# Plachtaa/FAcodec

Measured on NVIDIA H100. Metric: audio_seconds_per_second, higher is better.
Workload: dtype f32 I/O and accumulation; every product is a 3-MMA split of fp32 operands: fp16 hi + 2^11-scaled fp16 lo (22 mantissa bits, register-promoted accumulation) upstream of the VQ, bf16 hi + bf16 lo (16 bits) downstream

## Files before the change

### facodec_b200/_lib.py

```python
import ctypes
import os

from . import build as _build

_c = ctypes
_LIB = None


class FacError(RuntimeError):
    pass


def lib_path():
    return _build.LIB


def load():
    global _LIB
    if _LIB is not None:
        return _LIB
    path = lib_path()
    if not os.path.exists(path):
        raise FacError(f"{path} not found: build it with `python -m facodec_b200.build` "
                       "(needs nvcc; there is no CPU fallback)")
    L = ctypes.CDLL(path)
    vp, i32, i64p, fp = _c.c_void_p, _c.c_int, _c.c_void_p, _c.c_void_p
    sigs = {
        "fac_abi_version": ([], i32),
        "fac_create": ([_c.POINTER(vp), i32], i32),
        "fac_destroy": ([vp], i32),
        "fac_last_error": ([vp], _c.c_char_p),
        "fac_load_tensor": ([vp, i32, _c.c_char_p, fp, _c.POINTER(_c.c_int64), i32], i32),
        "fac_finalize": ([vp], i32),
        "fac_encode": ([vp, fp, i32, i32, fp, vp], i32),
        "fac_encode_frames": ([i32], i32),
        "fac_quantize": ([vp, fp, fp, i32, i32, i32, i32, fp, i32, i64p, fp, fp, fp, fp, fp, fp, i64p, i64p, i64p, vp], i32),
        "fac_decode": ([vp, fp, i32, i32, fp, vp], i32),
        "fac_codec_forward": ([vp, fp, i32, i32, i32, fp, i64p, i64p, i64p, fp, vp], i32),
        "fac_codec_forward_host": ([vp, fp, i32, i32, i32, fp, i64p, i64p, i64p, vp], i32),
        "fac_codec_encode": ([vp, fp, i32, i32, i32, i64p, i64p, i64p, fp, vp], i32),
        "fac_codec_encode_lens": ([vp, fp, i32, i32, vp, i32, i64p, i64p, i64p, fp, vp], i32),
        "fac_codec_forward_lens": ([vp, fp, i32, i32, vp, i32, fp, i64p, i64p, i64p, fp, vp], i32),
        "fac_codec_timbre_lens": ([vp, fp, i32, i32, vp, fp, vp], i32),
        "fac_dequantize": ([vp, i64p, i64p, i32, i64p, i32, fp, i32, i32, fp, fp, fp, fp, vp], i32),
        "fac_codes_decode": ([vp, i64p, i64p, i32, i64p, i32, fp, i32, i32, fp, vp], i32),
        "fac_codes_decode_lens": ([vp, i64p, i64p, i32, i64p, i32, fp, i32, i32, vp, fp, vp], i32),
        "fac_redecode": ([vp, i64p, i64p, i32, fp, i32, i32, i32, i32, i32, fp, vp], i32),
        "fac_redecoder_decode": ([vp, fp, i32, i32, fp, vp], i32),
        "fac_voice_convert": ([vp, i64p, i64p, i32, fp, i32, i32, i32, i32, i32, fp, vp], i32),
        "fac_voice_convert_lens": ([vp, i64p, i64p, i32, fp, i32, i32, i32, i32, i32, vp, fp, vp], i32),
        "fac_dataset_mel": ([vp, fp, i32, i32, fp, vp], i32),
        "fac_head_begin": ([vp], i32),
        "fac_head_tensor": ([vp, i32, _c.c_char_p, fp, _c.POINTER(_c.c_int64), i32], i32),
        "fac_head_finalize": ([vp, i32, i32, i32, i32, i32], i32),
        "fac_head_forward": ([vp, i32, fp, i32, i32, _c.POINTER(vp), vp], i32),
        "fac_rvq_create": ([vp, i32] + [_c.POINTER(vp)] * 5, i32),
        "fac_rvq_destroy": ([vp, i32], i32),
        "fac_stream_begin": ([vp, i32], i32),
        "fac_stream_encode": ([vp, i32, fp, i32, fp, vp], i32),
        "fac_stream_decode": ([vp, i32, fp, i32, fp, vp], i32),
        "fac_stream_decode_codes": ([vp, i32, i64p, i64p, i32, i64p, i32, fp, i32, fp, vp], i32),
        "fac_stream_encode_codes": ([vp, i32, fp, i32, i32, i64p, i64p, i64p, vp], i32),
        "fac_stream_finish_codes": ([vp, i32, i64p, i64p, i64p, fp, vp], i32),
        "fac_stream_timbre": ([vp, i32, fp, vp], i32),
        "fac_stream_end": ([vp, i32], i32),
        "fac_vc_stream_lookahead": ([], i32),
        "fac_vc_stream_begin": ([vp, i32, fp, i32, i32, i32, vp], i32),
        "fac_vc_stream_convert": ([vp, i32, i64p, i64p, i32, i32, fp, vp], i32),
        "fac_vc_stream_finish": ([vp, i32, fp, vp], i32),
        "fac_vc_stream_set_timbre": ([vp, i32, fp, vp], i32),
        "fac_vc_stream_end": ([vp, i32], i32),
        "fac_codes_pool_create": ([vp, i32, i32], i32),
        "fac_codes_pool_open": ([vp, i32, vp], i32),
        "fac_codes_pool_encode_codes": ([vp, i32, i32, vp, vp, vp, vp, vp, vp, vp, vp], i32),
        "fac_codes_pool_finish_codes": ([vp, i32, i32, vp, vp, vp, vp, vp, vp], i32),
        "fac_codes_pool_timbre": ([vp, i32, i32, vp, vp, vp], i32),
        "fac_codes_pool_close": ([vp, i32, i32], i32),
        "fac_codes_pool_destroy": ([vp, i32], i32),
        "fac_vc_pool_create": ([vp, i32, i32, i32, i32], i32),
        "fac_vc_pool_open": ([vp, i32, fp, vp], i32),
        "fac_vc_pool_open_mode": ([vp, i32, fp, i32, i32, i32, vp], i32),
        "fac_vc_pool_set_timbre": ([vp, i32, i32, fp, vp], i32),
        "fac_vc_pool_convert": ([vp, i32, i32, vp, vp, vp, vp, vp, vp, vp, vp], i32),
        "fac_vc_pool_finish": ([vp, i32, i32, vp, vp, vp, vp], i32),
        "fac_vc_pool_close": ([vp, i32, i32], i32),
        "fac_vc_pool_destroy": ([vp, i32], i32),
        "fac_dec_pool_create": ([vp, i32], i32),
        "fac_dec_pool_open": ([vp, i32, fp, vp], i32),
        "fac_dec_pool_decode_codes": ([vp, i32, i32, vp, vp, vp, vp, vp, vp, vp, vp, vp], i32),
        "fac_dec_pool_set_timbre": ([vp, i32, i32, fp, vp], i32),
        "fac_dec_pool_close": ([vp, i32, i32], i32),
        "fac_dec_pool_destroy": ([vp, i32], i32),
        "fac_resample_geometry": ([i32, i32, _c.POINTER(_c.c_int)], i32),
        "fac_resample_out_len": ([i32, i32, _c.c_longlong], _c.c_longlong),
        "fac_resample_ready": ([i32, i32, i32, _c.c_longlong, _c.c_longlong], _c.c_longlong),
        "fac_resample_table": ([vp, i32, i32, fp], i32),
        "fac_resample": ([vp, fp, i32, i32, vp, i32, i32, fp, vp], i32),
        "fac_rs_pool_create": ([vp, i32, i32], i32),
        "fac_rs_pool_open": ([vp, i32, i32, i32], i32),
        "fac_rs_pool_push": ([vp, i32, i32, vp, vp, vp, vp, vp, vp], i32),
        "fac_rs_pool_finish": ([vp, i32, i32, vp, vp, vp, vp, vp, vp], i32),
        "fac_rs_pool_undo": ([vp, i32, i32, vp], i32),
        "fac_rs_pool_close": ([vp, i32, i32], i32),
        "fac_rs_pool_destroy": ([vp, i32], i32),
# ... 68 lines not shown
```

### facodec_b200/build.py

```python
import os
import subprocess
import sys

HERE = os.path.dirname(os.path.abspath(__file__))
CSRC = os.path.join(HERE, "csrc")
OUT_DIR = os.path.join(HERE, "_C")
LIB = os.path.join(OUT_DIR, "libfacodec_b200.so")
SOURCES = ["engine.cu", "conv_simt.cu", "conv_tc.cu", "lstm.cu", "lstm2.cu", "frontend.cu", "quant.cu", "altfree.cu", "pool.cu", "resample.cu"]
HEADERS = ["common.cuh", "kernels.h", "conv_tc_common.cuh", "resample.h", os.path.join("..", "..", "include", "facodec_b200.h"),
           os.path.join("..", "..", "include", "facodec_b200_debug.h")]
NVCC_FLAGS = ["-O3", "-std=c++17", "-lineinfo", "-gencode", "arch=compute_90a,code=sm_90a",
              "-Xcompiler", "-fPIC", "-Xcompiler", "-O3", "--expt-relaxed-constexpr"]


def _nvcc():
    for c in (os.environ.get("NVCC"), "/usr/local/cuda/bin/nvcc", "nvcc"):
        if c and (os.path.isabs(c) and os.path.exists(c) or not os.path.isabs(c)):
            return c
    return "nvcc"


def is_stale():
    if not os.path.exists(LIB):
        return True
    t = os.path.getmtime(LIB)
    deps = [os.path.join(CSRC, s) for s in SOURCES + HEADERS] + [os.path.abspath(__file__)]
    return any(os.path.getmtime(d) > t for d in deps if os.path.exists(d))


def build(force=False, verbose=False):
    if not force and not is_stale():
        return LIB
    os.makedirs(OUT_DIR, exist_ok=True)
    objs = []
    procs = []
    for s in SOURCES:
        obj = os.path.join(OUT_DIR, s.replace(".cu", ".o"))
        cmd = [_nvcc()] + NVCC_FLAGS + (["-Xptxas", "-v"] if verbose else []) + ["-c", os.path.join(CSRC, s), "-o", obj]
        procs.append((s, subprocess.Popen(cmd, stdout=subprocess.PIPE, stderr=subprocess.STDOUT, text=True)))
        objs.append(obj)
    fail = False
    for s, p in procs:
        out, _ = p.communicate()
        if p.returncode != 0 or verbose:
            sys.stderr.write(f"--- {s} ---\n{out}\n")
        fail |= p.returncode != 0
    if fail:
        raise RuntimeError("nvcc failed")
    cmd = [_nvcc(), "-shared", "-o", LIB] + objs + ["-gencode", "arch=compute_90a,code=sm_90a", "-lcudart"]
    subprocess.check_call(cmd)
    return LIB


if __name__ == "__main__":
    print(build(force="--force" in sys.argv, verbose="-v" in sys.argv))
```

### facodec_b200/csrc/conv_tc.cu

```cuda
#include <cuda_bf16.h>
#include <cuda_fp16.h>

#include <cstring>
#include <mutex>
#include <type_traits>

#include "common.cuh"
#include "conv_tc_common.cuh"
#include "kernels.h"

namespace fac {

namespace {

using namespace tc;

enum Prec { P_TF32 = 0, P_BF16 = 1, P_F16S = 2, P_F16X2 = 3, P_NONE = -1 };

template <int P> struct PrecT {
    static constexpr int KG = P == P_TF32 ? 4 : 2;
    static constexpr int planes = P == P_F16S ? 1 : 2;
    static constexpr int ksteps = P == P_TF32 ? 2 : 1;
    static constexpr int kind = P == P_TF32 ? WG_TF32 : (P == P_BF16 ? WG_BF16 : WG_F16);
};

__host__ __device__ constexpr int prec_kg(int P) { return P == P_TF32 ? 4 : 2; }
__host__ __device__ constexpr int prec_planes(int P) { return P == P_F16S ? 1 : 2; }
__host__ __device__ constexpr uint32_t master_bytes(bool promoted, int nchunk, int promote_every, int ni) {
    return promoted && nchunk > promote_every ? (uint32_t)ni / 2 * 4 * kThreads : 0u;
}

template <int NI>
__device__ __forceinline__ void zero_acc(float (&a)[NI / 2]) {
#pragma unroll
    for (int i = 0; i < NI / 2; ++i) a[i] = 0.f;
}

template <int P, int NI>
__device__ __forceinline__ void mma_pass(float (&acc)[NI / 2], uint32_t a_addr, uint32_t a_lbo, uint32_t b_addr,
                                         uint32_t b_lbo) {
#pragma unroll
    for (int ks = 0; ks < PrecT<P>::ksteps; ++ks)
        wgmma_ss<NI, PrecT<P>::kind>(acc, gdesc(a_addr + ks * 2 * a_lbo, a_lbo, 128), gdesc(b_addr + ks * 2 * b_lbo, b_lbo, 128));
}

struct Tile {
    int row0, col0, nw;
    int warp, lane;
};

template <int NI, int GROUP = NI, typename F>
__device__ __forceinline__ void for_each_pair(const Tile& tl, const float (&acc)[NI / 2], F&& f) {
#pragma unroll
    for (int j = 0; j < NI / 8; ++j) {
        if (j > 0 && (8 * j) % GROUP == 0 && 8 * j >= tl.nw) break;
#pragma unroll
        for (int h = 0; h < 2; ++h) {
            const int row = tl.row0 + 16 * tl.warp + (tl.lane >> 2) + 8 * h;
            const int col = tl.col0 + 8 * j + 2 * (tl.lane & 3);
            f(row, col, acc[4 * j + 2 * h], acc[4 * j + 2 * h + 1]);
        }
    }
}

template <bool FAST>
__device__ __forceinline__ float act_out(int act, float v, float al, float ia) {
    if (act == ACT_SNAKE) return FAST ? fmaf(ia, sin2_mufu(al * v), v) : snake_fast(v, al, ia);
    if (act == ACT_TANH) return tanhf(v);
    if (act == ACT_MISH) return mish_f(v);
    return v;
}

template <int P1, int P2, bool TT>
constexpr bool groupable() { return P1 != P_F16S && P2 == P_NONE && !TT; }

template <int P1, int P2, bool PROMO, int NI, int MINB = 1, bool TT = false>
__global__ void __launch_bounds__(kThreads, groupable<P1, P2, TT>() && NI <= 128 ? 2 : MINB) conv_tc_kernel(TcConvParams p) {
    constexpr bool FUSED = P2 != P_NONE;
    constexpr bool GROUPABLE = groupable<P1, P2, TT>();
    static_assert(!TT || (NI == 64 && !FUSED), "transposed tiles: <= 64 channels x 64 time steps per warpgroup");
    static_assert(NI % 16 == 0 && NI <= (PROMO || MINB == 2 ? 64 : (P1 == P_F16S ? 256 : 128)),
                  "accumulator registers: <= 64 / 128 columns (256 in the one-pass fp16 class at one CTA per SM)");
    constexpr bool F16X2 = P1 == P_F16X2;
    constexpr bool DEC = P1 == P_BF16 || P1 == P_F16S;
    using T1 = PrecT<P1>;
    extern __shared__ __align__(1024) uint8_t smem[];
    uint64_t* full = reinterpret_cast<uint64_t*>(smem);

    const int tid = threadIdx.x, wg = tid >> 7;
    const int BM = 64 * p.MT;
    const int N = p.N, NW = p.MT == 2 ? N : N / 2;
    Tile tl;
    tl.row0 = p.MT == 2 ? 64 * wg : 0;
    tl.col0 = p.MT == 2 ? 0 : wg * NW;
    tl.nw = NW;
    tl.warp = (tid >> 5) & 3;
    tl.lane = tid & 31;
    const int t0 = blockIdx.x * BM, ntile = blockIdx.y, b = blockIdx.z;
    const int Kr = p.Kr, dil = p.dil, Rpad = p.Rpad, nchunk = p.nchunk, S = p.stagesB;
    const int G = GROUPABLE ? p.group : 1;
    const int R = BM + (Kr - 1) * dil;
    const int nstep1 = G == 4 ? nchunk >> 2 : (G == 2 ? nchunk >> 1 : nchunk);
    const uint32_t a_plane = (uint32_t)G * T1::KG * Rpad * 16, a_bytes = a_plane * T1::planes;
    uint8_t* abuf = smem + kSmemHdr;
    float4* master = reinterpret_cast<float4*>(abuf + 2 * (size_t)a_bytes);
    const uint32_t m_bytes = master_bytes(PROMO, nchunk, p.promote_every, NI);
    uint8_t* wbuf = abuf + 2 * (size_t)a_bytes + m_bytes;
    uint8_t* a2buf = m_bytes ? reinterpret_cast<uint8_t*>(master) : wbuf + (size_t)S * p.b_slot;
    const uint32_t w_unit1 = (uint32_t)Kr * T1::planes * T1::KG * N * 16;
    const uint32_t w_unit2 = FUSED ? (uint32_t)prec_planes(P2) * prec_kg(P2) * N * 16 : 0;
    const int units = nstep1 + (FUSED ? p.nchunk2 : 0);

    if (tid == 0) {
        for (int i = 0; i < S; ++i) mbar_init(&full[i], 1);
        fence_mbar_init();
    }
    __syncthreads();
    auto issue_w = [&](int u) {
        uint64_t* bar = &full[u % S];
        uint8_t* dst = wbuf + (size_t)(u % S) * p.b_slot;
        const uint8_t* src;
        uint32_t bytes;
        if (u < nstep1) {
            src = reinterpret_cast<const uint8_t*>(p.wblob) + ((size_t)ntile * nchunk + (size_t)u * G) * w_unit1;
            bytes = G * w_unit1;
        } else { src = reinterpret_cast<const uint8_t*>(p.wblob2) + (size_t)(u - nstep1) * w_unit2; bytes = w_unit2; }
        mbar_arrive_expect_tx(bar, bytes);
        bulk_g2s(dst, src, bytes, bar);
    };
    if (tid == 0)
        for (int u = 0; u < S - 1 && u < units; ++u) issue_w(u);

    const PadMap pm = PadMap::lane(p.lane_len, b, p.Tin, p.pad_left_s, p.pad_right_s, p.reflect);
    const float* __restrict__ xb = p.x + (size_t)b * p.x_bstride;
    auto produce = [&](int s) {
        uint8_t* ahi = abuf + (size_t)(s & 1) * a_bytes;
        auto run = [&](auto grouped) {
            constexpr bool GR = decltype(grouped)::value;
            const int c = GR ? s * G : s;
            if constexpr (P1 == P_TF32) produce_chunk<kThreads, GR, false>(p, pm, xb, c, G, t0, R, Rpad, ahi, ahi + a_plane, tid);
            else if constexpr (P1 == P_BF16) produce_chunk<kThreads, GR, true>(p, pm, xb, c, G, t0, R, Rpad, ahi, ahi + a_plane, tid);
            else if constexpr (P1 == P_F16S) produce_chunk<kThreads, GR, true, 4, false, false, true>(p, pm, xb, c, G, t0, R, Rpad, ahi, ahi, tid);
            else produce_chunk<kThreads, GR, false, 4, false, true>(p, pm, xb, c, G, t0, R, Rpad, ahi, ahi + a_plane, tid);
        };
        if constexpr (GROUPABLE) {
            if (G > 1) run(std::true_type());
            else run(std::false_type());
        } else {
            run(std::false_type());
        }
        fence_proxy_async();
    };
    produce(0);

    float acc[NI / 2];
    float crs[F16X2 ? NI / 2 : 1];
    zero_acc<NI>(acc);
    if constexpr (F16X2) zero_acc<NI>(crs);
    const uint32_t a_lbo = (uint32_t)Rpad * 16, b_lbo = (uint32_t)N * 16;
    const uint32_t abase = smem_u32(abuf), wbase = smem_u32(wbuf), a2base = smem_u32(a2buf);
    const int BM2 = BM;

    auto promote = [&](bool first, bool last) {
        if constexpr (PROMO) {
#pragma unroll
            for (int q = 0; q < NI / 8; ++q) {
                float w[4];
#pragma unroll
                for (int e = 0; e < 4; ++e) {
                    const int i = 4 * q + e;
                    if constexpr (F16X2) { w[e] = acc[i] + crs[i] * kLoUnscale; crs[i] = 0.f; }
                    else w[e] = acc[i];
                }
                float4 m = first ? make_float4(0.f, 0.f, 0.f, 0.f) : master[q * kThreads + tid];
                m.x += w[0]; m.y += w[1]; m.z += w[2]; m.w += w[3];
                if (!last) master[q * kThreads + tid] = m;
                acc[4 * q + 0] = last ? m.x : 0.f;
                acc[4 * q + 1] = last ? m.y : 0.f;
                acc[4 * q + 2] = last ? m.z : 0.f;
                acc[4 * q + 3] = last ? m.w : 0.f;
            }
        }
    };

#pragma unroll 1
    for (int u = 0; u < units; ++u) {
        __syncthreads();
        if (tid == 0 && u + S - 1 < units) issue_w(u + S - 1);
        mbar_wait(&full[u % S], (uint32_t)(u / S) & 1u);
        const uint32_t wslot = wbase + (uint32_t)(u % S) * p.b_slot;
        wg_fence();
        if (u < nstep1) {
            const uint32_t a0 = abase + (uint32_t)(u & 1) * a_bytes + (uint32_t)tl.row0 * 16;
            const uint32_t b0 = wslot + (uint32_t)tl.col0 * 16;
            auto mma_tap = [&](uint32_t ahi, uint32_t bhi) {
                const uint32_t alo = ahi + a_plane, blo = bhi + T1::KG * b_lbo;
                if constexpr (TT) {
                    mma_pass<P1, NI>(acc, bhi, b_lbo, ahi, a_lbo);
                    mma_pass<P1, NI>(crs, bhi, b_lbo, alo, a_lbo);
                    mma_pass<P1, NI>(crs, blo, b_lbo, ahi, a_lbo);
                } else if constexpr (P1 == P_F16S) {
                    mma_pass<P1, NI>(acc, ahi, a_lbo, bhi, b_lbo);
                } else if constexpr (F16X2) {
                    mma_pass<P1, NI>(acc, ahi, a_lbo, bhi, b_lbo);
                    mma_pass<P1, NI>(crs, ahi, a_lbo, blo, b_lbo);
                    mma_pass<P1, NI>(crs, alo, a_lbo, bhi, b_lbo);
                } else {
                    mma_pass<P1, NI>(acc, ahi, a_lbo, bhi, b_lbo);
                    mma_pass<P1, NI>(acc, ahi, a_lbo, blo, b_lbo);
                    mma_pass<P1, NI>(acc, alo, a_lbo, bhi, b_lbo);
                }
            };
            if constexpr (GROUPABLE) {
                uint32_t ac = a0, bc = b0, ahi = a0, bhi = b0;
#pragma unroll 1
                for (int i = 0, tap = 0; i < G * Kr; ++i) {
                    mma_tap(ahi, bhi);
                    if (++tap < Kr) { ahi += (uint32_t)dil * 16; bhi += T1::planes * T1::KG * b_lbo; }
                    else { tap = 0; ac += T1::KG * a_lbo; bc += w_unit1; ahi = ac; bhi = bc; }
                }
            } else {
#pragma unroll 1
                for (int tap = 0; tap < Kr; ++tap)
                    mma_tap(a0 + (uint32_t)(tap * dil) * 16, b0 + (uint32_t)tap * T1::planes * T1::KG * b_lbo);
            }
            wg_commit();
            if (u + 1 < nstep1) produce(u + 1);
            wg_wait_all();
            const int done = (u + 1) * G;
            if (PROMO && (done % p.promote_every == 0 || done == nchunk)) promote(done <= p.promote_every, done == nchunk);
            if constexpr (FUSED) {
                if (u + 1 == nstep1) {
                    constexpr int KG2 = prec_kg(P2 < 0 ? 0 : P2);
                    const uint32_t a2_plane = (uint32_t)(p.nchunk2 * KG2) * BM2 * 16;
                    if (m_bytes) __syncthreads();
                    for_each_pair<NI, 32>(tl, acc, [&](int row, int col, float v0, float v1) {
                        const float2 bi = __ldg(reinterpret_cast<const float2*>(p.bias + col));
                        const float2 al = __ldg(reinterpret_cast<const float2*>(p.out_alpha + col));
                        const float2 ia = __ldg(reinterpret_cast<const float2*>(p.out_inv_alpha + col));
                        v0 = act_out<DEC>(ACT_SNAKE, v0 + bi.x, al.x, ia.x);
                        v1 = act_out<DEC>(ACT_SNAKE, v1 + bi.y, al.y, ia.y);
                        if constexpr (P2 == P_BF16) {
                            __nv_bfloat162 h = __floats2bfloat162_rn(v0, v1);
                            float2 hf = __bfloat1622float2(h);
                            __nv_bfloat162 l = __floats2bfloat162_rn(v0 - hf.x, v1 - hf.y);
                            const uint32_t off = ((uint32_t)(col >> 3) * BM2 + row) * 16 + (col & 7) * 2;
                            *reinterpret_cast<__nv_bfloat162*>(a2buf + off) = h;
                            *reinterpret_cast<__nv_bfloat162*>(a2buf + a2_plane + off) = l;
                        } else if constexpr (P2 == P_F16X2) {
                            const __half2 h = __floats2half2_rn(v0, v1);
                            const float2 hf = __half22float2(h);
                            const __half2 l = __floats2half2_rn((v0 - hf.x) * kLoScale, (v1 - hf.y) * kLoScale);
                            const uint32_t off = ((uint32_t)(col >> 3) * BM2 + row) * 16 + (col & 7) * 2;
                            *reinterpret_cast<__half2*>(a2buf + off) = h;
                            *reinterpret_cast<__half2*>(a2buf + a2_plane + off) = l;
                        } else {
                            const float h0 = to_tf32(v0), h1 = to_tf32(v1);
                            const uint32_t off = ((uint32_t)(col >> 2) * BM2 + row) * 16 + (col & 3) * 4;
                            *reinterpret_cast<float2*>(a2buf + off) = make_float2(h0, h1);
                            *reinterpret_cast<float2*>(a2buf + a2_plane + off) = make_float2(to_tf32(v0 - h0), to_tf32(v1 - h1));
                        }
                    });
                    fence_proxy_async();
                    zero_acc<NI>(acc);
                }
            }
        } else if constexpr (FUSED) {
            constexpr int P2x = P2 < 0 ? 0 : P2;
            constexpr int KG2 = prec_kg(P2x);
            const int c2 = u - nstep1;
            const uint32_t a2_plane = (uint32_t)(p.nchunk2 * KG2) * BM2 * 16, a2_lbo = (uint32_t)BM2 * 16;
            const uint32_t ahi = a2base + ((uint32_t)(c2 * KG2) * BM2 + tl.row0) * 16, alo = ahi + a2_plane;
            const uint32_t bhi = wslot + (uint32_t)tl.col0 * 16, blo = bhi + KG2 * b_lbo;
            if constexpr (P2x == P_F16X2) {
                mma_pass<P2x, NI>(acc, ahi, a2_lbo, bhi, b_lbo);
                mma_pass<P2x, NI>(crs, ahi, a2_lbo, blo, b_lbo);
                mma_pass<P2x, NI>(crs, alo, a2_lbo, bhi, b_lbo);
            } else {
                mma_pass<P2x, NI>(acc, ahi, a2_lbo, bhi, b_lbo);
                mma_pass<P2x, NI>(acc, ahi, a2_lbo, blo, b_lbo);
                mma_pass<P2x, NI>(acc, alo, a2_lbo, bhi, b_lbo);
            }
            wg_commit();
            wg_wait_all();
            if (PROMO && c2 + 1 == p.nchunk2) promote(true, true);
        }
    }

    const float* __restrict__ bias = FUSED ? p.bias2 : p.bias;
    const int act = FUSED ? ACT_NONE : p.out_act;
    float* __restrict__ yb = p.y + (size_t)b * p.y_bstride + (size_t)ntile * N;
    const float* __restrict__ rb = p.res ? p.res + (size_t)b * p.y_bstride + (size_t)ntile * N : nullptr;
    const float* al_p = act == ACT_SNAKE ? p.out_alpha + (size_t)ntile * N : nullptr;
    const float* ia_p = act == ACT_SNAKE ? p.out_inv_alpha + (size_t)ntile * N : nullptr;
    const float* bi_p = bias ? bias + (size_t)ntile * N : nullptr;
    if constexpr (TT) {
        for_each_pair<NI>(tl, acc, [&](int r, int c, float v0, float v1) {
            if (r - tl.row0 >= NW) return;
            const int co = tl.col0 + (r - tl.row0), tf = tl.row0 + (c - tl.col0);
            const float bi = bi_p ? __ldg(bi_p + co) : 0.f;
            const float al = act == ACT_SNAKE ? __ldg(al_p + co) : 0.f, ia = act == ACT_SNAKE ? __ldg(ia_p + co) : 0.f;
            const float v[2] = {v0, v1};
#pragma unroll
            for (int e = 0; e < 2; ++e) {
                const int t = t0 + tf + e;
                if (t >= p.Tout) continue;
                float o = act_out<DEC>(act, v[e] + bi, al, ia);
                if (rb) o += rb[(size_t)t * p.ldy + co];
                yb[(size_t)t * p.ldy + co] = o;
            }
        });
        return;
    }
    for_each_pair<NI>(tl, acc, [&](int row, int col, float v0, float v1) {
        const int t = t0 + row;
        if (t >= p.Tout) return;
        if (bi_p) { const float2 bi = __ldg(reinterpret_cast<const float2*>(bi_p + col)); v0 += bi.x; v1 += bi.y; }
        if (act == ACT_SNAKE) {
            const float2 al = __ldg(reinterpret_cast<const float2*>(al_p + col));
            const float2 ia = __ldg(reinterpret_cast<const float2*>(ia_p + col));
            v0 = act_out<DEC>(ACT_SNAKE, v0, al.x, ia.x);
            v1 = act_out<DEC>(ACT_SNAKE, v1, al.y, ia.y);
        } else if (act != ACT_NONE) {
            v0 = act_out<DEC>(act, v0, 0.f, 0.f);
            v1 = act_out<DEC>(act, v1, 0.f, 0.f);
        }
        if (rb) { const float2 r = *reinterpret_cast<const float2*>(rb + (size_t)t * p.ldy + col); v0 += r.x; v1 += r.y; }
        *reinterpret_cast<float2*>(yb + (size_t)t * p.ldy + col) = make_float2(v0, v1);
    });
}

}

namespace {
constexpr size_t kSmemCap = 227 * 1024;
constexpr size_t kSmemCap2 = 113 * 1024;
int plan_prec(const TcConvParams& p) {
    return p.g1f16 ? P_F16S : (p.f16x2 ? P_F16X2 : (p.bf16 ? P_BF16 : P_TF32));
}
constexpr int f16s_wide_nw(bool fused) { return fused ? 192 : 256; }
}

bool tc_conv_plan(TcConvParams& p) {
    if ((p.Cin % 4) != 0 || ((p.Cin * p.vf) % kChunk) != 0 || (p.Cout % 16) != 0) return false;
    if (p.bf16 && p.promoted) return false;
    if (p.f16x2 && !p.promoted) return false;
    if (p.g1f16 && !p.bf16) return false;
    if (p.tt && !p.f16x2) return false;
    if (p.fused && ((p.promoted && (!p.f16x2 || p.tt)) || p.Cin != p.Cout || p.vf != 1 || p.Cout > 256)) return false;
    const int P1 = plan_prec(p), P2 = p.fused ? (p.f16x2 ? P_F16X2 : (p.bf16 ? P_BF16 : P_TF32)) : P_NONE;
    p.nchunk = p.Cin * p.vf / kChunk;
    p.nchunk2 = p.fused ? p.Cout / kChunk : 0;
    p.promote_every = p.promoted ? (p.f16x2 ? (48 / p.Kr < 1 ? 1 : 48 / p.Kr) : (8 / p.Kr < 1 ? 1 : 8 / p.Kr)) : 1;
    if (p.fused && p.promoted && p.nchunk2 > 48) return false;
    const int nw_max = p.promoted ? 64 : 128;
    constexpr size_t kAReserve = 40 * 1024;
    int N = 0;
    for (int cand = p.fused ? p.Cout : 256; cand >= 16 && N == 0; cand -= 16) {
        const bool rows_split = cand <= nw_max, cols_split = (cand / 2) % 16 == 0 && cand / 2 <= nw_max;
        if (p.Cout % cand || !(rows_split || cols_split)) continue;
        size_t slot = (size_t)p.Kr * prec_planes(P1) * prec_kg(P1) * cand * 16, a2 = 0;
        if (P2 != P_NONE) a2 = (size_t)prec_planes(P2) * p.nchunk2 * prec_kg(P2) * 64 * 16;
        if (kSmemHdr + kAReserve + slot + a2 <= kSmemCap) N = cand;
        else if (p.fused) return false;
    }
    if (N == 0 || (p.fused && p.promoted && N != p.Cout)) return false;
    struct Layout { int Rpad; size_t slot, total; };
    auto layout = [&](int S, int MT, int G) {
        const int NW = MT == 2 ? N : N / 2, BM = 64 * MT;
        Layout l;
        const int v = G == 1 ? 2 : (P1 == P_TF32 ? 1 : 4 / G);
        l.Rpad = BM + (p.Kr - 1) * p.dil;
        while (l.Rpad % 8 != v) ++l.Rpad;
        const size_t a_bytes = (size_t)G * prec_planes(P1) * prec_kg(P1) * l.Rpad * 16;
        l.slot = (size_t)G * p.Kr * prec_planes(P1) * prec_kg(P1) * N * 16;
        size_t a2 = 0;
        if (P2 != P_NONE) {
            const size_t slot2 = (size_t)prec_planes(P2) * prec_kg(P2) * N * 16;
            if (slot2 > l.slot) l.slot = slot2;
            a2 = (size_t)prec_planes(P2) * p.nchunk2 * prec_kg(P2) * BM * 16;
        }
        const size_t master = master_bytes(p.promoted, p.nchunk, p.promote_every, p.tt ? 64 : NW);
        if (master) a2 = 0;
        l.total = kSmemHdr + 2 * a_bytes + master + S * l.slot + a2 + (p.tt ? 64 * 16 : 0);
        return l;
    };
    auto group = [&](int S, int MT, size_t cap) {
        if (p.Kr > 3 || p.tt || p.fused || p.g1f16) return 1;
        for (int G = 4; G > 1; G /= 2)
            if (G <= p.max_group && p.nchunk % G == 0 && (!p.promoted || p.promote_every % G == 0) && layout(S, MT, G).total <= cap) return G;
        return 1;
    };
    const bool unit2 = p.fused && p.promoted;
    const bool want2 = p.promoted ? !p.tt : (p.occ2_maxn > 0 && N <= p.occ2_maxn);
    for (int two = want2 ? 1 : 0; two >= (unit2 ? 1 : 0); --two) {
        const size_t cap = two ? kSmemCap2 : kSmemCap;
        const int nwl = two ? 64 : nw_max;
        for (int S = 2; S >= 1; --S)
            for (int MT = 2; MT >= 1; --MT) {
                const int NW = MT == 2 ? N : N / 2;
                const bool wide = !two && P1 == P_F16S && NW == f16s_wide_nw(p.fused);
                if ((NW > nwl && !wide) || NW % 16 || (unit2 && NW != 64)) continue;
                if (wide && layout(2, 1, 1).total <= kSmemCap2) continue;
                const Layout l1 = layout(S, MT, 1);
                if (l1.total > cap) continue;
                const int G = group(S, MT, l1.total <= kSmemCap2 ? kSmemCap2 : cap);
                const Layout l = layout(S, MT, G);
                p.N = N; p.MT = MT; p.Rpad = l.Rpad; p.R2pad = 64 * MT; p.stagesB = S; p.b_slot = (int)l.slot;
                p.group = G;
                p.smem_bytes = l.total;
                p.occ2 = two;
                return true;
            }
    }
    return false;
}

size_t tc_blob_floats(const TcConvParams& p) {
    if (p.g1f16) return (size_t)(p.Cout / p.N) * p.nchunk * p.Kr * 2 * p.N * 4;
    return (size_t)(p.Cout / p.N) * p.nchunk * p.Kr * 2 * ((p.bf16 || p.f16x2) ? 2 : 4) * p.N * 4;
}

static inline uint16_t bf16_rn_host(float f) {
    uint32_t u;
    memcpy(&u, &f, 4);
    u += 0x7FFFu + ((u >> 16) & 1u);
    return (uint16_t)(u >> 16);
}

void tc_pack_blob(const TcConvParams& p, const float* wp, int ldw, float* blob) {
    const int Cw = p.Cin * p.vf;
    if (p.g1f16) {
        uint16_t* ob = reinterpret_cast<uint16_t*>(blob);
        size_t o16 = 0;
        for (int nt = 0; nt < p.Cout / p.N; ++nt)
            for (int c = 0; c < p.nchunk; ++c)
                for (int tap = 0; tap < p.Kr; ++tap)
                    for (int k8 = 0; k8 < 2; ++k8)
                        for (int n = 0; n < p.N; ++n)
                            for (int e = 0; e < 8; ++e) {
                                int kk = tap * Cw + c * tc::kChunk + k8 * 8 + e;
                                __half v = __float2half_rn(wp[(size_t)kk * ldw + nt * p.N + n]);
                                uint16_t bits;
                                memcpy(&bits, &v, 2);
                                ob[o16++] = bits;
                            }
        return;
    }
    if (p.f16x2) {
        uint16_t* ob = reinterpret_cast<uint16_t*>(blob);
        size_t o16 = 0;
        for (int nt = 0; nt < p.Cout / p.N; ++nt)
            for (int c = 0; c < p.nchunk; ++c)
                for (int tap = 0; tap < p.Kr; ++tap)
                    for (int hl = 0; hl < 2; ++hl)
                        for (int k8 = 0; k8 < 2; ++k8)
                            for (int n = 0; n < p.N; ++n)
                                for (int e = 0; e < 8; ++e) {
                                    int kk = tap * Cw + c * tc::kChunk + k8 * 8 + e;
                                    float w = wp[(size_t)kk * ldw + nt * p.N + n];
                                    __half hi = __float2half_rn(w);
                                    __half v = hl == 0 ? hi : __float2half_rn((w - __half2float(hi)) * 2048.0f);
                                    uint16_t bits;
                                    memcpy(&bits, &v, 2);
                                    ob[o16++] = bits;
                                }
        return;
    }
    if (p.bf16) {
        uint16_t* ob = reinterpret_cast<uint16_t*>(blob);
        size_t o16 = 0;
        for (int nt = 0; nt < p.Cout / p.N; ++nt)
            for (int c = 0; c < p.nchunk; ++c)
                for (int tap = 0; tap < p.Kr; ++tap)
                    for (int hl = 0; hl < 2; ++hl)
                        for (int k8 = 0; k8 < 2; ++k8)
                            for (int n = 0; n < p.N; ++n)
                                for (int e = 0; e < 8; ++e) {
                                    int kk = tap * Cw + c * tc::kChunk + k8 * 8 + e;
                                    float w = wp[(size_t)kk * ldw + nt * p.N + n];
                                    uint16_t hi = bf16_rn_host(w);
                                    uint32_t hu = (uint32_t)hi << 16;
                                    float hf;
                                    memcpy(&hf, &hu, 4);
                                    ob[o16++] = hl == 0 ? hi : bf16_rn_host(w - hf);
                                }
        return;
    }
    size_t o = 0;
    for (int nt = 0; nt < p.Cout / p.N; ++nt)
        for (int c = 0; c < p.nchunk; ++c)
            for (int tap = 0; tap < p.Kr; ++tap)
                for (int hl = 0; hl < 2; ++hl)
                    for (int k4 = 0; k4 < 4; ++k4)
                        for (int n = 0; n < p.N; ++n)
                            for (int e = 0; e < 4; ++e) {
                                int kk = tap * Cw + c * tc::kChunk + k4 * 4 + e;
                                float w = wp[(size_t)kk * ldw + nt * p.N + n];
                                uint32_t u;
                                memcpy(&u, &w, 4);
// ... 75 lines not shown
```

### facodec_b200/csrc/engine.cu

```cuda
#include <cmath>
#include <cstdio>
#include <cstdlib>
#include <cstring>
#include <algorithm>
#include <initializer_list>
#include <map>
#include <memory>
#include <string>
#include <type_traits>
#include <vector>

#include "../../include/facodec_b200.h"
#include "../../include/facodec_b200_debug.h"
#include "common.cuh"
#include "kernels.h"
#include "resample.h"

using namespace fac;

namespace {

constexpr int HOP = 300;
constexpr int LATENT = 1024;
constexpr int N_FFT = 2048;
// ... 4073 lines not shown
    return n;
}

int fac_debug_pad_map(int L, int pad_left, int pad_right, int reflect, int* out, int n) {
    if (!out || L < 0 || pad_left < 0 || pad_right < 0 || n != pad_left + L + pad_right) return FAC_ERR_INVALID;
    const PadMap pm = PadMap::make(L, pad_left, pad_right, reflect);
    for (int i = 0; i < n; ++i) out[i] = pm.src(i - pad_left);
    return FAC_OK;
}

int fac_debug_lane_pad_map(const int* lane_len, int B, int Tin, int pad_left, int pad_right, int reflect, int* out, int n) {
    if (!out || B <= 0 || Tin < 0 || pad_left < 0 || pad_right < 0 || n != pad_left + Tin + pad_right) return FAC_ERR_INVALID;
    for (int b = 0; lane_len && b < B; ++b)
        if (lane_len[b] < 0 || lane_len[b] > Tin) return FAC_ERR_INVALID;
    for (int b = 0; b < B; ++b) {
        const PadMap pm = PadMap::lane(lane_len, b, Tin, pad_left, pad_right, reflect);
        for (int i = 0; i < n; ++i) out[(size_t)b * n + i] = pm.src(i - pad_left);
    }
    return FAC_OK;
}

static int debug_tc_plan(int Cin, int Cout, int K, int dil, int stride, int Tout, int mode, int occ2_maxn, TcConvParams& tp) {
    if (Cin <= 0 || Cout <= 0 || K <= 0 || dil <= 0 || stride <= 0 || mode < 0 || mode > 9) return FAC_ERR_INVALID;
    tp.Cin = Cin; tp.Cout = Cout; tp.Tout = Tout; tp.occ2_maxn = occ2_maxn;
    tp.promoted = (mode == 1 || mode == 3 || mode == 9) ? 1 : 0;
    tp.bf16 = (mode == 2 || mode == 4 || mode == 7 || mode == 8) ? 1 : 0;
    tp.f16x2 = (mode == 3 || mode == 9) ? 1 : 0;
    tp.fused = (mode == 4 || mode == 5 || mode == 8 || mode == 9) ? 1 : 0;
    tp.g1f16 = (mode == 7 || mode == 8) ? 1 : 0;
    if (mode == 6) { tp.promoted = 1; tp.f16x2 = 1; tp.tt = 1; }
    if (stride == 1) { tp.vf = 1; tp.Kr = K; tp.dil = dil; }
    else if (K == 2 * stride && dil == 1) { tp.vf = stride; tp.Kr = 2; tp.dil = 1; }
    else return FAC_ERR_UNSUPPORTED;
    return tc_conv_plan(tp) ? FAC_OK : FAC_ERR_UNSUPPORTED;
}

int fac_debug_tc_plan(int Cin, int Cout, int K, int dil, int stride, int Tout, int mode, int occ2_maxn, int* out8) {
    if (!out8) return FAC_ERR_INVALID;
    TcConvParams tp;
    const int rc = debug_tc_plan(Cin, Cout, K, dil, stride, Tout, mode, occ2_maxn, tp);
    if (rc != FAC_OK) return rc;
    out8[0] = tp.N; out8[1] = tp.MT; out8[2] = tp.nchunk; out8[3] = tp.stagesB; out8[4] = tp.R2pad;
    out8[5] = (int)tp.smem_bytes; out8[6] = tp.Rpad; out8[7] = tp.promote_every;
    return FAC_OK;
}

int fac_debug_tc_plan_group(int Cin, int Cout, int K, int dil, int stride, int Tout, int mode, int occ2_maxn, int* smem2) {
    TcConvParams tp;
    const int rc = debug_tc_plan(Cin, Cout, K, dil, stride, Tout, mode, occ2_maxn, tp);
    if (rc != FAC_OK) return rc;
    if (smem2) {
        TcConvParams t1 = tp;
        t1.max_group = 1;
        if (!tc_conv_plan(t1)) return FAC_ERR_UNSUPPORTED;
        smem2[0] = (int)tp.smem_bytes;
        smem2[1] = (int)t1.smem_bytes;
    }
    return tp.group;
}

long long fac_debug_tc_pack(const float* w_host, int Cin, int Cout, int K, int stride, int mode, float* blob_out,
                            long long capacity_floats) {
    if (!w_host || Cin <= 0 || Cout <= 0 || K <= 0 || stride <= 0 || mode < 0 || mode > 3) return FAC_ERR_INVALID;
    TcConvParams tp;
    tp.Cin = Cin; tp.Cout = Cout; tp.dil = 1;
    tp.promoted = (mode == 1 || mode == 3) ? 1 : 0; tp.bf16 = mode == 2 ? 1 : 0; tp.f16x2 = mode == 3 ? 1 : 0;
    if (stride == 1) { tp.vf = 1; tp.Kr = K; }
    else if (K == 2 * stride) { tp.vf = stride; tp.Kr = 2; }
    else return FAC_ERR_UNSUPPORTED;
    if (!tc_conv_plan(tp)) return FAC_ERR_UNSUPPORTED;
    const long long n = (long long)tc_blob_floats(tp);
    if (!blob_out || capacity_floats < n) return n;
    const int ldw = (Cout + 3) / 4 * 4;
    std::vector<float> gen((size_t)K * Cin * ldw, 0.f);
    for (int co = 0; co < Cout; ++co)
        for (int ci = 0; ci < Cin; ++ci)
            for (int k = 0; k < K; ++k) gen[((size_t)k * Cin + ci) * ldw + co] = w_host[((size_t)co * Cin + ci) * K + k];
    tc_pack_blob(tp, gen.data(), ldw, blob_out);
    return n;
}

int fac_debug_tc_phase_clocks(fac_handle* h, long long* out8) {
    if (!h || !out8) return FAC_ERR_INVALID;
    h->err = "fac_debug_tc_phase_clocks: the tensor-core conv kernel records no timing probes";
    return FAC_ERR_UNSUPPORTED;
}

int fac_debug_tc_trace(fac_handle* h, long long* out80) {
    if (!h || !out80) return FAC_ERR_INVALID;
    h->err = "fac_debug_tc_trace: the tensor-core conv kernel records no timing probes";
    return FAC_ERR_UNSUPPORTED;
}

int fac_debug_tc_producer_clocks(fac_handle* h, long long* out4) {
    if (!h || !out4) return FAC_ERR_INVALID;
    h->err = "fac_debug_tc_producer_clocks: the tensor-core conv kernel records no timing probes";
    return FAC_ERR_UNSUPPORTED;
}

int fac_debug_lstm_phase_clocks(fac_handle* h, long long* out4) {
    if (!h || !out4) return FAC_ERR_INVALID;
    cudaSetDevice(h->device);
    cudaDeviceSynchronize();
    cudaError_t e = h->lstm_v2 ? lstm2_read_phase_clocks(out4) : lstm_read_phase_clocks(out4);
    if (e != cudaSuccess) { h->err = cudaGetErrorString(e); return FAC_ERR_CUDA; }
    return FAC_OK;
}

int fac_debug_tap(fac_handle* h, const char* name, float* dst, size_t capacity_floats) {
    if (!h || !name) return FAC_ERR_INVALID;
    if (!dst) h->taps.erase(name);
    else h->taps[name] = std::make_pair(dst, capacity_floats);
    return FAC_OK;
}

int fac_profile_enable(fac_handle* h, int on) {
    if (!h) return FAC_ERR_INVALID;
    h->profiling = on != 0;
    return FAC_OK;
}

static void profile_collect(fac_handle* h) {
    if (h->prof.empty()) return;
    cudaSetDevice(h->device);
    cudaDeviceSynchronize();
    for (auto& r : h->prof) {
        float ms = 0.f;
        cudaEventElapsedTime(&ms, r.a, r.b);
        auto& a = h->prof_agg[r.name];
        a.ms += ms; a.flops += r.flops; a.bytes += r.bytes; a.launches++;
        cudaEventDestroy(r.a); cudaEventDestroy(r.b);
    }
    h->prof.clear();
}

int fac_profile_reset(fac_handle* h) {
    if (!h) return FAC_ERR_INVALID;
    profile_collect(h);
    h->prof_agg.clear();
    return FAC_OK;
}

int fac_profile_get(fac_handle* h, const char* family, double* ms, double* flops, double* bytes, long long* launches) {
    if (!h || !family) return FAC_ERR_INVALID;
    profile_collect(h);
    std::string fam(family);
    fac_handle::ProfAgg t;
    for (auto& kv : h->prof_agg) {
        if (kv.first == fam || (kv.first.size() > fam.size() && kv.first.compare(0, fam.size(), fam) == 0 && kv.first[fam.size()] == ':')) {
            t.ms += kv.second.ms; t.flops += kv.second.flops; t.bytes += kv.second.bytes; t.launches += kv.second.launches;
        }
    }
    if (ms) *ms = t.ms;
    if (flops) *flops = t.flops;
    if (bytes) *bytes = t.bytes;
    if (launches) *launches = t.launches;
    return FAC_OK;
}

size_t fac_profile_dump(fac_handle* h, char* buf, size_t cap) {
    if (!h) return 0;
    profile_collect(h);
    std::string out;
    char line[256];
    for (auto& kv : h->prof_agg) {
        snprintf(line, sizeof line, "%s\t%.4f\t%.3f\t%.4f\t%ld\n", kv.first.c_str(), kv.second.ms, kv.second.flops / 1e9,
                 kv.second.bytes / 1e9, kv.second.launches);
        out += line;
// ... 14 lines not shown
```

### facodec_b200/csrc/kernels.h

```cpp
#pragma once
#include <cuda_runtime.h>
#include <stdint.h>

namespace fac {

struct ConvParams {
    const float* x = nullptr;
    const float* w = nullptr;
    const float* bias = nullptr;
    const float* in_alpha = nullptr;
    const float* in_inv_alpha = nullptr;
    const float* out_alpha = nullptr;
    const float* out_inv_alpha = nullptr;
    const float* res = nullptr;
    const int* valid_len = nullptr;
    const int* lane_len = nullptr;
    float* y = nullptr;
    int B = 0, Tin = 0, Cin = 0, Tout = 0, Cout = 0;
    int K = 1, dil = 1, stride = 1, pad_left = 0, pad_right = 0, pad_reflect = 0;
    int ldw = 0, ldy = 0, ldx = 0;
    int out_act = 0;
    int y_transposed = 0;
    size_t x_bstride = 0, y_bstride = 0;
};
cudaError_t launch_conv(const ConvParams& p, cudaStream_t st);

struct TcConvParams {
    const float* x = nullptr;
    const float* wblob = nullptr;
    const float* bias = nullptr;
    const float* in_alpha = nullptr;
    const float* in_inv_alpha = nullptr;
    const float* out_alpha = nullptr;
    const float* out_inv_alpha = nullptr;
    const float* res = nullptr;
    float* y = nullptr;
    int B = 0, Tin = 0, Cin = 0, ldx = 0;
    int vf = 1;
    int Kr = 1, dil = 1, PLr = 0;
    int pad_left_s = 0, pad_right_s = 0, reflect = 0;
    const int* lane_len = nullptr;
    int Tout = 0, Cout = 0, ldy = 0;
    int out_act = 0;
    int promoted = 0;
    int bf16 = 0;
    int g1f16 = 0;
    int f16x2 = 0;
    int fused = 0;
    int tt = 0;
    int occ2_maxn = 0;
    int max_group = 4;
    const float* wblob2 = nullptr;
    const float* bias2 = nullptr;
    int nchunk2 = 0;
    int promote_every = 1;
    int N = 0, nchunk = 0, Rpad = 0, stagesB = 0;
    int group = 1;
    int MT = 2;
    int b_slot = 0;
    int occ2 = 0;
    int R2pad = 0;
    size_t smem_bytes = 0;
    size_t x_bstride = 0, y_bstride = 0;
};
bool tc_conv_plan(TcConvParams& p);
size_t tc_blob_floats(const TcConvParams& p);
void tc_pack_blob(const TcConvParams& p, const float* wp, int ldw, float* blob);
cudaError_t launch_conv_tc(const TcConvParams& p, cudaStream_t st);

struct LstmParams {
    const float* xg = nullptr;
    const float* whh_p = nullptr;
    const float* whh_p16 = nullptr;
    int bf16 = 0;
    const uint32_t* whh_p2 = nullptr;
    uint32_t* h16 = nullptr;
    int pass3 = 0;
    uint32_t* state_h = nullptr;
    float* state_c = nullptr;
    const float* skip = nullptr;
    float* y = nullptr;
    float* hT = nullptr;
    unsigned int* bar = nullptr;
    int B = 0, T = 0, H = 0, U = 0, G = 0;
};
struct LstmLaneLens { int len[32]; };
cudaError_t launch_lstm_layer(const LstmParams& p, cudaStream_t st);
cudaError_t launch_lstm2_layer(const LstmParams& p, cudaStream_t st, const LstmLaneLens* lens = nullptr);
size_t lstm2_pack_words(int H, int U, int pass3);
void lstm2_pack(const float* whh, int H, int U, int pass3, uint32_t* out);
size_t lstm2_smem_bytes(int H, int U, int pass3);
void lstm2_state_sizes(int H, int U, int pass3, size_t* h_words, size_t* c_floats);
cudaError_t lstm2_read_phase_clocks(long long* out4);
void lstm2_lane_map(int H, int U, int pass3, int b, long long* pos);
constexpr int kLaneMax = 32;
struct LaneCarryParams {
    uint32_t* slot[kLaneMax];
    uint32_t* state_h = nullptr;
    float* state_c = nullptr;
    int n = 0, H = 0, U = 0, pass3 = 0, to_lanes = 0;
};
cudaError_t launch_lstm2_lane_carry(const LaneCarryParams& p, cudaStream_t st);
struct LaneCopyParams {
    const uint32_t* src[kLaneMax];
    uint32_t* dst[kLaneMax];
    long long words[kLaneMax];
    int n = 0;
};
cudaError_t launch_lane_copy(const LaneCopyParams& p, cudaStream_t st);
int lstm_units_per_cta(int H);
cudaError_t lstm_read_phase_clocks(long long* out4);

cudaError_t launch_stft_frames(const float* wave, float* frames , int B, int T, int F, int hop, int win, int pad,
                               cudaStream_t st, int f_first = 0, const int* lane_len = nullptr);
cudaError_t launch_mel_from_spec(const float* spec, int ldspec, const float* fb , float* mel,
                                 int B, int F, int Tm, cudaStream_t st);

struct VqWeights {
    const float* w_in;
    const float* b_in;
    const float* cb;
    const float* cbn;
    const float* cbn2;
    const float* w_out;
    const float* b_out;
};
struct FaqParams {
    const float* f0 = nullptr;
    const float* z = nullptr;
    VqWeights vq[6];
    int n_c = 1;
    const float* gamma_beta = nullptr;
    float* outs = nullptr;
    float* zp = nullptr, *zc = nullptr, *zr = nullptr;
    int64_t* codes_p = nullptr;
    int64_t* codes_c = nullptr;
    int64_t* codes_r = nullptr;
    float* sqerr = nullptr;
    int B = 0, Tq = 0, Tz = 0, Tf0 = 0;
};
cudaError_t launch_fa_quantize(const FaqParams& p, cudaStream_t st);
cudaError_t launch_fa_codes(const FaqParams& p, cudaStream_t st);
struct DeqParams {
    const int64_t* codes_p = nullptr;
    const int64_t* codes_c = nullptr;
    const int64_t* codes_r = nullptr;
    int n_c = 1, n_r = 3;
    VqWeights vq[6];
    const float* gamma_beta = nullptr;
    float* outs = nullptr;
    float* zp = nullptr, *zc = nullptr, *zr = nullptr;
// ... 59 lines not shown
```

Baseline: 1057.

## Deepen weight prefetch in promoted TC conv and add phase-clock probe

In the promoted-accumulation tensor-core conv path, the kernel now preloads all S weight slots up front. Each slot is refilled only after the warpgroup MMAs on it have completed, using an extra barrier, instead of issuing the next load at the top of each iteration. Producing the next activation tile also moves to after the MMA wait in that path, which gives up overlap between activation staging and the MMAs in exchange for a deeper weight pipeline. It also adds a compile-time-gated clock64 phase probe, a debug readout API, and build options for out-of-tree builds with extra defines.

Result: no change. 1066 (median of 6 runs) (+0.9%).

```diff
diff --git a/facodec_b200/_lib.py b/facodec_b200/_lib.py
--- a/facodec_b200/_lib.py
+++ b/facodec_b200/_lib.py
@@ -15,11 +15,13 @@
     return _build.LIB
 
 
-def load():
+def load(path=None):
     global _LIB
     if _LIB is not None:
+        if path is not None and path != _LIB._name:
+            raise FacError(f"{_LIB._name} is already loaded")
         return _LIB
-    path = lib_path()
+    path = path or lib_path()
     if not os.path.exists(path):
         raise FacError(f"{path} not found: build it with `python -m facodec_b200.build` "
                        "(needs nvcc; there is no CPU fallback)")
diff --git a/facodec_b200/build.py b/facodec_b200/build.py
--- a/facodec_b200/build.py
+++ b/facodec_b200/build.py
@@ -28,15 +28,18 @@
     return any(os.path.getmtime(d) > t for d in deps if os.path.exists(d))
 
 
-def build(force=False, verbose=False):
-    if not force and not is_stale():
+def build(force=False, verbose=False, out_dir=None, defines=()):
+    if out_dir is None and not force and not is_stale():
         return LIB
-    os.makedirs(OUT_DIR, exist_ok=True)
+    out_dir = out_dir or OUT_DIR
+    lib = os.path.join(out_dir, os.path.basename(LIB))
+    os.makedirs(out_dir, exist_ok=True)
     objs = []
     procs = []
     for s in SOURCES:
-        obj = os.path.join(OUT_DIR, s.replace(".cu", ".o"))
-        cmd = [_nvcc()] + NVCC_FLAGS + (["-Xptxas", "-v"] if verbose else []) + ["-c", os.path.join(CSRC, s), "-o", obj]
+        obj = os.path.join(out_dir, s.replace(".cu", ".o"))
+        cmd = [_nvcc()] + NVCC_FLAGS + [f"-D{d}" for d in defines] + (["-Xptxas", "-v"] if verbose else []) + \
+            ["-c", os.path.join(CSRC, s), "-o", obj]
         procs.append((s, subprocess.Popen(cmd, stdout=subprocess.PIPE, stderr=subprocess.STDOUT, text=True)))
         objs.append(obj)
     fail = False
@@ -47,10 +50,19 @@
         fail |= p.returncode != 0
     if fail:
         raise RuntimeError("nvcc failed")
-    cmd = [_nvcc(), "-shared", "-o", LIB] + objs + ["-gencode", "arch=compute_90a,code=sm_90a", "-lcudart"]
+    cmd = [_nvcc(), "-shared", "-o", lib] + objs + ["-gencode", "arch=compute_90a,code=sm_90a", "-lcudart"]
     subprocess.check_call(cmd)
-    return LIB
+    return lib
 
 
 if __name__ == "__main__":
-    print(build(force="--force" in sys.argv, verbose="-v" in sys.argv))
+    import argparse
+    ap = argparse.ArgumentParser()
+    ap.add_argument("--force", action="store_true")
+    ap.add_argument("-v", dest="verbose", action="store_true")
+    ap.add_argument("--out", default=None, help="build into this directory instead of facodec_b200/_C")
+    ap.add_argument("-D", dest="defines", action="append", default=[], help="preprocessor macro (with --out)")
+    a = ap.parse_args()
+    if a.defines and not a.out:
+        ap.error("-D needs --out: the in-tree library is the shipped build")
+    print(build(force=a.force, verbose=a.verbose, out_dir=a.out, defines=a.defines))
diff --git a/facodec_b200/csrc/conv_tc.cu b/facodec_b200/csrc/conv_tc.cu
--- a/facodec_b200/csrc/conv_tc.cu
+++ b/facodec_b200/csrc/conv_tc.cu
@@ -74,8 +74,23 @@
 template <int P1, int P2, bool TT>
 constexpr bool groupable() { return P1 != P_F16S && P2 == P_NONE && !TT; }
 
+#ifdef FAC_TC_PHASE_PROBE
+__device__ unsigned long long g_tc_phase_clock[8];
+#define TC_PHASE(i)                                                         \
+    do {                                                                    \
+        const long long n_ = clock64();                                     \
+        ph_[i] += n_ - ph_t_;                                               \
+        ph_t_ = n_;                                                         \
+    } while (0)
+#else
+#define TC_PHASE(i) do { } while (0)
+#endif
+
 template <int P1, int P2, bool PROMO, int NI, int MINB = 1, bool TT = false>
 __global__ void __launch_bounds__(kThreads, groupable<P1, P2, TT>() && NI <= 128 ? 2 : MINB) conv_tc_kernel(TcConvParams p) {
+#ifdef FAC_TC_PHASE_PROBE
+    long long ph_[7] = {}, ph_t_ = clock64();
+#endif
     constexpr bool FUSED = P2 != P_NONE;
     constexpr bool GROUPABLE = groupable<P1, P2, TT>();
     static_assert(!TT || (NI == 64 && !FUSED), "transposed tiles: <= 64 channels x 64 time steps per warpgroup");
@@ -129,7 +144,8 @@
         bulk_g2s(dst, src, bytes, bar);
     };
     if (tid == 0)
-        for (int u = 0; u < S - 1 && u < units; ++u) issue_w(u);
+        for (int u = 0; u < (PROMO ? S : S - 1) && u < units; ++u) issue_w(u);
+    TC_PHASE(0);
 
     const PadMap pm = PadMap::lane(p.lane_len, b, p.Tin, p.pad_left_s, p.pad_right_s, p.reflect);
     const float* __restrict__ xb = p.x + (size_t)b * p.x_bstride;
@@ -152,6 +168,7 @@
         fence_proxy_async();
     };
     produce(0);
+    TC_PHASE(3);
 
     float acc[NI / 2];
     float crs[F16X2 ? NI / 2 : 1];
@@ -161,6 +178,10 @@
     const uint32_t abase = smem_u32(abuf), wbase = smem_u32(wbuf), a2base = smem_u32(a2buf);
     const int BM2 = BM;
 
+    auto refill = [&](int u) {
+        __syncthreads();
+        if (tid == 0 && u + S < units) issue_w(u + S);
+    };
     auto promote = [&](bool first, bool last) {
         if constexpr (PROMO) {
 #pragma unroll
@@ -186,8 +207,10 @@
 #pragma unroll 1
     for (int u = 0; u < units; ++u) {
         __syncthreads();
-        if (tid == 0 && u + S - 1 < units) issue_w(u + S - 1);
+        TC_PHASE(0);
+        if (!PROMO && tid == 0 && u + S - 1 < units) issue_w(u + S - 1);
         mbar_wait(&full[u % S], (uint32_t)(u / S) & 1u);
+        TC_PHASE(1);
         const uint32_t wslot = wbase + (uint32_t)(u % S) * p.b_slot;
         wg_fence();
         if (u < nstep1) {
@@ -225,8 +248,19 @@
                     mma_tap(a0 + (uint32_t)(tap * dil) * 16, b0 + (uint32_t)tap * T1::planes * T1::KG * b_lbo);
             }
             wg_commit();
-            if (u + 1 < nstep1) produce(u + 1);
+            TC_PHASE(2);
+            if constexpr (!PROMO) {
+                if (u + 1 < nstep1) produce(u + 1);
+                TC_PHASE(3);
+            }
             wg_wait_all();
+            TC_PHASE(4);
+            if constexpr (PROMO) {
+                refill(u);
+                TC_PHASE(1);
+                if (u + 1 < nstep1) produce(u + 1);
+                TC_PHASE(3);
+            }
             const int done = (u + 1) * G;
             if (PROMO && (done % p.promote_every == 0 || done == nchunk)) promote(done <= p.promote_every, done == nchunk);
             if constexpr (FUSED) {
@@ -282,11 +316,27 @@
                 mma_pass<P2x, NI>(acc, alo, a2_lbo, bhi, b_lbo);
             }
             wg_commit();
+            TC_PHASE(2);
             wg_wait_all();
+            TC_PHASE(4);
+            if constexpr (PROMO) {
+                refill(u);
+                TC_PHASE(1);
+            }
             if (PROMO && c2 + 1 == p.nchunk2) promote(true, true);
         }
-    }
-
+        TC_PHASE(5);
+    }
+
+    auto probe_flush = [&]() {
+#ifdef FAC_TC_PHASE_PROBE
+        TC_PHASE(6);
+        if (PROMO && tid == 0) {
+            for (int i = 0; i < 7; ++i) atomicAdd(&g_tc_phase_clock[i], (unsigned long long)ph_[i]);
+            atomicAdd(&g_tc_phase_clock[7], 1ull);
+        }
+#endif
+    };
     const float* __restrict__ bias = FUSED ? p.bias2 : p.bias;
     const int act = FUSED ? ACT_NONE : p.out_act;
     float* __restrict__ yb = p.y + (size_t)b * p.y_bstride + (size_t)ntile * N;
@@ -310,6 +360,7 @@
                 yb[(size_t)t * p.ldy + co] = o;
             }
         });
+        probe_flush();
         return;
     }
     for_each_pair<NI>(tl, acc, [&](int row, int col, float v0, float v1) {
@@ -328,6 +379,7 @@
         if (rb) { const float2 r = *reinterpret_cast<const float2*>(rb + (size_t)t * p.ldy + col); v0 += r.x; v1 += r.y; }
         *reinterpret_cast<float2*>(yb + (size_t)t * p.ldy + col) = make_float2(v0, v1);
     });
+    probe_flush();
 }
 
 }
@@ -416,6 +468,20 @@
     return false;
 }
 
+cudaError_t tc_read_phase_clocks(long long* out8) {
+#ifdef FAC_TC_PHASE_PROBE
+    unsigned long long v[8];
+    cudaError_t e = cudaMemcpyFromSymbol(v, g_tc_phase_clock, sizeof(v));
+    if (e != cudaSuccess) return e;
+    for (int i = 0; i < 8; ++i) out8[i] = (long long)v[i];
+    const unsigned long long zero[8] = {};
+    return cudaMemcpyToSymbol(g_tc_phase_clock, zero, sizeof(zero));
+#else
+    (void)out8;
+    return cudaErrorNotSupported;
+#endif
+}
+
 size_t tc_blob_floats(const TcConvParams& p) {
     if (p.g1f16) return (size_t)(p.Cout / p.N) * p.nchunk * p.Kr * 2 * p.N * 4;
     return (size_t)(p.Cout / p.N) * p.nchunk * p.Kr * 2 * ((p.bf16 || p.f16x2) ? 2 : 4) * p.N * 4;
diff --git a/facodec_b200/csrc/engine.cu b/facodec_b200/csrc/engine.cu
--- a/facodec_b200/csrc/engine.cu
+++ b/facodec_b200/csrc/engine.cu
@@ -4179,8 +4179,15 @@
 
 int fac_debug_tc_phase_clocks(fac_handle* h, long long* out8) {
     if (!h || !out8) return FAC_ERR_INVALID;
-    h->err = "fac_debug_tc_phase_clocks: the tensor-core conv kernel records no timing probes";
-    return FAC_ERR_UNSUPPORTED;
+    cudaSetDevice(h->device);
+    cudaDeviceSynchronize();
+    const cudaError_t e = tc_read_phase_clocks(out8);
+    if (e == cudaErrorNotSupported) {
+        h->err = "fac_debug_tc_phase_clocks: the library was compiled without FAC_TC_PHASE_PROBE";
+        return FAC_ERR_UNSUPPORTED;
+    }
+    if (e != cudaSuccess) { h->err = cudaGetErrorString(e); return FAC_ERR_CUDA; }
+    return FAC_OK;
 }
 
 int fac_debug_tc_trace(fac_handle* h, long long* out80) {
diff --git a/facodec_b200/csrc/kernels.h b/facodec_b200/csrc/kernels.h
--- a/facodec_b200/csrc/kernels.h
+++ b/facodec_b200/csrc/kernels.h
@@ -67,6 +67,7 @@
 size_t tc_blob_floats(const TcConvParams& p);
 void tc_pack_blob(const TcConvParams& p, const float* wp, int ldw, float* blob);
 cudaError_t launch_conv_tc(const TcConvParams& p, cudaStream_t st);
+cudaError_t tc_read_phase_clocks(long long* out8);
 
 struct LstmParams {
     const float* xg = nullptr;
```
